# lkeegan/blockCG

Hardware: AMD Instinct MI355X
Metric: SBCGrQ lattice-site iterations/sec (iterations/sec x global volume), fp64 (higher is better)
Workload: dtype f64; 1 GPU; SBCGrQ V=64x64x64x64 (64x64x64x64 per GPU), m=16, 4 shifts, mass=0.001, fixed-work (eps=0); m=16, transport=none, half_volume_solves=False, memory_ladder_rung=whole tmp

## Files before the change

### blockcg_amd/csrc/capi_context.hip

```cpp
#include "capi_internal.hpp"

namespace bcg_impl {

std::string g_create_error;

void resolve_profile(bcg_context* c) {
  for (auto& kv : c->prof) {
    for (auto& pr : kv.second.pending) {
      float ms = 0.f;
      if (hipEventElapsedTime(&ms, pr.first, pr.second) == hipSuccess) {
        kv.second.ms += ms;
        kv.second.count += 1;
      }
      c->event_pool.push_back(pr.first);
      c->event_pool.push_back(pr.second);
    }
    kv.second.pending.clear();
  }
}

int stream_sync(bcg_context* c) {
  HIP_TRY(c, hipStreamSynchronize(c->stream));
  c->mat_in_flight = 0;
  if (c->profiling) resolve_profile(c);
// ... 327 lines not shown
  c->lat.ndim = ndim;
  c->lat.V = V;
  for (int mu = 0; mu < 4; ++mu) {
    c->lat.face_sites[mu] = V / c->lat.L[mu];
    c->lat.ghost_off[mu][0] = c->lat.ghost_off[mu][1] = 0;
    if (c->lat.split[mu]) {
      c->lat.ghost_off[mu][0] = ghost;
      c->lat.ghost_off[mu][1] = ghost + c->lat.face_sites[mu];
      ghost += 2 * c->lat.face_sites[mu];
    }
  }
  c->ghost_sites = ghost;
  if (const char* e = std::getenv("BCG_ROW_BLOCKS_B")) c->row_blocks_B = std::atoi(e);
  if (const char* e = std::getenv("BCG_ROW_BLOCKS_C")) c->row_blocks_C = std::atoi(e);
  if (const char* e = std::getenv("BCG_ROW_BATCHED")) c->row_batched = std::atoi(e) != 0;
  if (const char* e = std::getenv("BCG_HOP_WALK")) c->hop_tune.patch_walk = std::atoi(e) != 0;
  if (const char* e = std::getenv("BCG_HOP_BLOCKS")) c->hop_tune.blocks = std::atoi(e);
  if (const char* e = std::getenv("BCG_HOP_BLOCKS_OVERLAP")) c->hop_tune.blocks_overlap = std::atoi(e);
  if (const char* e = std::getenv("BCG_HOP_SUPER")) c->hop_tune.super_patch = std::atoi(e);
  if (const char* e = std::getenv("BCG_HOP_SYNC")) c->hop_tune.sync.window = std::atoi(e);
  if (const char* e = std::getenv("BCG_HOP_SYNC_LIMIT")) c->hop_tune.sync.limit_ticks = std::atoi(e);
  if (const char* e = std::getenv("BCG_HOP_COLUMN")) c->hop_tune.sync.column_walk = std::atoi(e) != 0;
  if (const char* e = std::getenv("BCG_HOP_BUNDLE")) c->hop_tune.sync.bundle_walk = std::atoi(e);
  if (const char* e = std::getenv("BCG_HOP_BUNDLE_SYNC")) c->hop_tune.sync.bundle_window = std::atoi(e);
  if (const char* e = std::getenv("BCG_LAZY_Q")) c->lazy_q = std::atoi(e);
  if (const char* e = std::getenv("BCG_PAIR_SHIFTS")) c->pair_shifts = std::atoi(e);
  if (const char* e = std::getenv("BCG_DEFER_X0")) c->defer_x0 = std::atoi(e) != 0;
  if (const char* e = std::getenv("BCG_DEBUG_X0_COND_LIMIT")) c->x0_cond_limit = std::atof(e);
  if (const char* e = std::getenv("BCG_RING_CHUNK")) c->ring_chunk_override = std::atoi(e);
  if (const char* e = std::getenv("BCG_DEBUG_FIELD_BUDGET")) c->debug_field_budget = static_cast<size_t>(std::atoll(e));
// ... 90 lines not shown
  if (!c) return BCG_ERR_INVALID;
  if (send) *send = c->halo_send;
  if (recv) *recv = c->halo_recv;
  if (bytes_each) *bytes_each = c->halo_bytes;
  return BCG_OK;
}

int bcg_debug_read_scratch(bcg_context* c, void* host, size_t bytes) {
  DeviceScope on_device(c);
  if (!c || !host || !c->partials || bytes > c->partials_bytes) return BCG_ERR_INVALID;
  BCG_TRY(stream_sync(c));
  HIP_TRY(c, hipMemcpy(host, c->partials, bytes, hipMemcpyDeviceToHost));
  return BCG_OK;
}

int bcg_context_stream(const bcg_context* c, void** stream_out, int* device_out) {
  if (!c) return BCG_ERR_INVALID;
  if (stream_out) *stream_out = c->stream;
  if (device_out) *device_out = c->device;
  return BCG_OK;
}

int bcg_overlap_tuning(bcg_context* c, int interior_blocks) {
  if (!c || interior_blocks < 0 || interior_blocks > kMaxGramBlocks / 2) return BCG_ERR_INVALID;
  if (interior_blocks > 0) c->hop_tune.blocks_overlap = interior_blocks;
  return BCG_OK;
}

int bcg_synchronize(bcg_context* c) {
  DeviceScope on_device(c);
// ... 325 lines not shown
```

### blockcg_amd/csrc/capi_internal.hpp

```cpp
#pragma once
#include <hip/hip_runtime.h>

#include <algorithm>
#include <cmath>
#include <cstdio>
#include <cstdlib>
#include <cstring>
#include <sstream>
#include <string>
#include <thread>
#include <vector>

#include "context.hpp"
#include "kernels_mfma.hpp"

#define BCG_FAIL(ctx, code, msg) \
  do {                           \
    (ctx)->err = (msg);          \
    return (code);               \
  } while (0)

#define HIP_TRY(ctx, call)                                                                         \
  do {                                                                                             \
    hipError_t e_ = (call);                                                                        \
// ... 20 lines not shown
  explicit DeviceScope(const bcg_context* c) {
    if (!c) return;
    if (hipGetDevice(&prev) == hipSuccess && prev != c->device) switched = hipSetDevice(c->device) == hipSuccess;
  }
  ~DeviceScope() {
    if (switched) (void)hipSetDevice(prev);
  }
  DeviceScope(const DeviceScope&) = delete;
  DeviceScope& operator=(const DeviceScope&) = delete;
};

struct ProfScope {
  bcg_context* c;
  bcg::ProfEntry* e = nullptr;
  hipEvent_t a = nullptr, b = nullptr;
  ProfScope(bcg_context* ctx, const char* name, double alg_bytes = 0.0, double alg_flops = 0.0) : c(ctx) {
    if (!c->profiling) return;
    e = &c->prof[name];
    e->bytes += alg_bytes;
    e->flops += alg_flops;
    a = take();
    b = take();
    (void)hipEventRecord(a, c->stream);
  }
  ~ProfScope() {
    if (!e) return;
    (void)hipEventRecord(b, c->stream);
    e->pending.emplace_back(a, b);
  }
  hipEvent_t take() {
    if (!c->event_pool.empty()) {
      hipEvent_t ev = c->event_pool.back();
      c->event_pool.pop_back();
      return ev;
    }
    hipEvent_t ev;
    (void)hipEventCreate(&ev);
    return ev;
  }
};

constexpr int kMaxGramBlocks = 2048;
constexpr size_t kMatSlotBytes = 32 * 32 * sizeof(double2);
constexpr int kMatSlots = 96;

constexpr int kFastBlocks = 1024;

inline int64_t rows_of(const bcg_field* f) { return f->sites * 3; }
inline double alg_bytes(const bcg_context* c, int m, double fields, double links = 0.0, int64_t num = 1, int64_t den = 1) {
  return static_cast<double>(c->lat.V) * (fields * 48.0 * m + links * 144.0 * c->ndim) * static_cast<double>(num) /
         static_cast<double>(den);
}
inline double row_bytes(const bcg_field* f, double fields) { return static_cast<double>(f->sites) * 48.0 * f->m * fields; }
inline double product_flops(const bcg_field* f, double products) {
  return static_cast<double>(f->sites) * 3.0 * f->m * f->m * 8.0 * products;
}
inline double hop_flops(const bcg_context* c, int m, bool gram, int64_t num = 1, int64_t den = 1) {
  return static_cast<double>(c->lat.V) * m * (72.0 * 2 * c->ndim + (gram ? 24.0 * m : 0.0)) * static_cast<double>(num) /
         static_cast<double>(den);
}
inline size_t field_bytes(const bcg_context* c, int m) { return static_cast<size_t>(c->lat.V) * 3 * m * sizeof(double2); }
// ... 21 lines not shown

int halo_plan(int ndim, const int* gdims, const int* grid, const int* coords, size_t site_bytes, int* peer_s, int* peer_r,
              size_t* off_s, size_t* off_r, size_t* nb, int64_t* ghost_sites);
inline bool can_overlap(const bcg_context* c) {
  return c->distributed && c->have_comm && c->comm.halo_exchange_begin && c->comm.halo_exchange_end;
}
int halo_field(bcg_context* c, const bcg_field* f, bool split = false);
int halo_gauge(bcg_context* c, bcg_gauge* g);
int hop(bcg_context* c, const bcg_gauge* g, bcg_field* out, const bcg_field* in, bcg::HopMode mode, const bcg_field* p, double c0,
        int* gram_blocks = nullptr, bool* gram_folded = nullptr);
int get_tmp(bcg_context* c, int m, bcg_field** out);
bool capacity_path(const bcg_context* c, int m);
inline bool ring_overlapped(const bcg_context* c) { return c->ring_overlap && can_overlap(c) && (c->tmp_ring - 2) / 2 >= 1; }
int reserve_operator_scratch(bcg_context* c, const bcg_field* like);
int apply_shifted(bcg_context* c, const bcg_gauge* g, double mass, double sigma0, bcg_field* T, const bcg_field* P,
                  int* gram_blocks = nullptr, bool* gram_folded = nullptr);

int pair_shifts_depth(const bcg_context* c, int m, int n_shifts);
int thin_qr(bcg_context* c, bcg_field* y, CMat& R);

}
```

### blockcg_amd/csrc/capi_operator.hip

```cpp
#include "capi_internal.hpp"

namespace bcg_impl {

int rank_of_grid(const int* grid, const int* xyz) {
  int r = 0, st = 1;
  for (int mu = 0; mu < 4; ++mu) {
    r += xyz[mu] * st;
    st *= grid[mu];
  }
  return r;
}

int halo_plan(int ndim, const int* gdims, const int* grid, const int* coords, size_t site_bytes, int* peer_s, int* peer_r,
              size_t* off_s, size_t* off_r, size_t* nb, int64_t* ghost_sites) {
  int g4[4] = {1, 1, 1, 1}, c4[4] = {0, 0, 0, 0}, L[4] = {1, 1, 1, 1};
  int64_t V = 1;
  for (int mu = 0; mu < ndim; ++mu) {
    g4[mu] = grid ? grid[mu] : 1;
    c4[mu] = coords ? coords[mu] : 0;
    if (g4[mu] < 1 || gdims[mu] < 1 || gdims[mu] % g4[mu] != 0 || c4[mu] < 0 || c4[mu] >= g4[mu]) return -1;
    L[mu] = gdims[mu] / g4[mu];
    V *= L[mu];
  }
  int n = 0;
// ... 445 lines not shown
  const int m = like->m;
  bcg_field* tmp;
  if (like->parity >= 0) {
    BCG_TRY(get_tmp_half(c, m, 1 - like->parity, &tmp));
    if (c->distributed) BCG_TRY(ensure_halo(c, static_cast<size_t>(c->ghost_sites) * 3 * m * sizeof(double2)));
    if (half_chunked_path(c) && fast_hop(c, m)) BCG_TRY(ensure_half_chunk_scratch(c, m));
    return BCG_OK;
  }
  if (fast_hop(c, m)) BCG_TRY(ensure_scratch(c));
  if (capacity_path(c, m)) return ensure_ring_scratch(c, m);
  BCG_TRY(get_tmp(c, m, &tmp));
  if (c->distributed) BCG_TRY(ensure_halo(c, static_cast<size_t>(c->ghost_sites) * 3 * m * sizeof(double2)));
  return BCG_OK;
}

int apply_shifted(bcg_context* c, const bcg_gauge* g, double mass, double sigma0, bcg_field* T, const bcg_field* P,
                  int* gram_blocks, bool* gram_folded) {
  if (gram_folded) *gram_folded = false;
  if (P->parity >= 0) {
    if (gram_blocks) *gram_blocks = 0;
    if (T->parity != P->parity) BCG_FAIL(c, BCG_ERR_INVALID, "half-volume operator: result and argument must have the same parity");
    const int m = P->m;
    bcg_field* tmp;
    BCG_TRY(get_tmp_half(c, m, 1 - P->parity, &tmp));
    BCG_TRY(halo_gauge(c, const_cast<bcg_gauge*>(g)));
    bcg::LatticeDev latc = c->lat;
    latc.L[0] /= 2;
    latc.V /= 2;
    for (int mu = 1; mu < 4; ++mu) latc.stride[mu] /= 2;
    for (int mu = 0; mu < 4; ++mu) {
      latc.face_sites[mu] /= 2;
      latc.ghost_off[mu][0] /= 2;
      latc.ghost_off[mu][1] /= 2;
// ... 56 lines not shown
      ProfScope ps(c, "hop_half", alg_bytes(c, m, 2, 2, 1, 2), hop_flops(c, m, false, 1, 2));
      bcg::launch_hop_half(c->stream, m, c->lat, tmp->parity, g->U, g->Ughost, P->d, c->halo_recv, tmp->d, bcg::HOP_PLAIN, nullptr, 0.0);
    }
    BCG_TRY(check_launch(c, "hop_half"));
    BCG_TRY(halo_field(c, tmp));
    {
      ProfScope ps(c, "hop_half_shifted", alg_bytes(c, m, 3, 2, 1, 2), hop_flops(c, m, false, 1, 2));
      bcg::launch_hop_half(c->stream, m, c->lat, T->parity, g->U, g->Ughost, tmp->d, c->halo_recv, T->d, bcg::HOP_SHIFTED, P->d,
                           mass * mass + sigma0);
    }
    return check_launch(c, "hop_half_shifted");
  }
  if (capacity_path(c, P->m)) return apply_shifted_ring(c, g, mass, sigma0, T, P, gram_blocks);
  bcg_field* tmp;
  BCG_TRY(get_tmp(c, P->m, &tmp));
  BCG_TRY(hop(c, g, tmp, P, bcg::HOP_PLAIN, nullptr, 0.0));
  return hop(c, g, T, tmp, bcg::HOP_SHIFTED, P, mass * mass + sigma0, gram_blocks, gram_folded);
}


}

using namespace bcg_impl;

extern "C" {

int bcg_halo_plan(int ndim, const int* global_dims, const int* grid, const int* coords, size_t site_bytes, int* peer_send,
                  int* peer_recv, size_t* send_offset, size_t* recv_offset, size_t* nbytes, int64_t* ghost_sites) {
  if (ndim < 1 || ndim > 4 || !global_dims || !peer_send || !peer_recv || !send_offset || !recv_offset || !nbytes) return -1;
  return halo_plan(ndim, global_dims, grid, coords, site_bytes, peer_send, peer_recv, send_offset, recv_offset, nbytes,
                   ghost_sites);
}
// ... 72 lines not shown
```

### blockcg_amd/csrc/capi_solvers.hip

```cpp
#include "capi_internal.hpp"

namespace bcg_impl {

int phase_A(bcg_context* c, const bcg_gauge* g, double mass, double sigma0, bcg_field* T, const bcg_field* P, CMat& G) {
  int nb = 0;
  bool folded = false;
  BCG_TRY(apply_shifted(c, g, mass, sigma0, T, P, &nb, &folded));
  if (nb > 0) return finish_gram(c, P->m, nb, G, true, folded);
  return gram(c, P, T, G);
}

int rmul(bcg_context* c, bcg_field* y, const bcg_field* x, const CMat& M, double b, bcg::RmulMode mode, const char* name);
bool lazy_q_width(const bcg_context* c, int m) {
  return c->lazy_q && fast_rows(c, m) && fast_rmul(c, m) && (m == 8 || m == 16 || (m == 32 && c->lazy_q > 1));
}

int phase_B(bcg_context* c, bcg_field* Q, const bcg_field* T, const CMat& alpha, CMat& G2, const CMat* rinv_prev = nullptr,
            bcg_field* Qout = nullptr) {
  const int m = Q->m;
  if (!fast_rows(c, m)) {
    if (Qout) BCG_FAIL(c, BCG_ERR_INVALID, "phase B: a separate output needs the fused kernel");
    BCG_TRY(rmul(c, Q, T, -alpha, 0.0, bcg::RMUL_ADD, "block_axpy"));
    return gram(c, Q, Q, G2);
  }
// ... 872 lines not shown
```

### blockcg_amd/csrc/context.hpp

```cpp
#pragma once
#include <hip/hip_runtime.h>

#include <map>
#include <string>
#include <vector>

#include "../../include/blockcg_hip.h"
#include "kernels.hpp"
#include "kernels_mfma.hpp"
#include "small_matrix.hpp"

struct bcg_field {
  bcg_context* ctx;
  int m;
  double2* d;
  void* base;
  int parity = -1;
  int64_t sites = 0;
};

struct bcg_gauge {
  bcg_context* ctx;
  double2* U;
  double2* Ughost;
// ... 18 lines not shown
  bool own_stream = false;
  int ndim = 1;
  int gdims[4] = {1, 1, 1, 1};
  int grid[4] = {1, 1, 1, 1};
  int coords[4] = {0, 0, 0, 0};
  bcg::LatticeDev lat{};
  int64_t ghost_sites = 0;
  bool distributed = false;
  bcg_comm comm{};
  bool have_comm = false;
  bool force_generic = false;
  bool force_tile_classes = false;
  int row_blocks_B = 1024, row_blocks_C = 1024;
  bool row_batched = true;
  bcg::HopTuning hop_tune;

  std::map<int, bcg_field*> tmp_field;
  int tmp_ring = 0;
  std::map<int, double2*> tmp_ring_buf;
  std::map<int, std::pair<int*, int>> boundary_tiles;
  double2* halo_send = nullptr;
  double2* halo_recv = nullptr;
  size_t halo_bytes = 0;
  void* halo_save = nullptr;
  size_t halo_save_bytes = 0;
  int lazy_q = 1;
  int pair_shifts = 4;
  bool defer_x0 = true;
  double x0_cond_limit = 64.0;
  size_t debug_field_budget = 0;
// ... 31 lines not shown
```

### blockcg_amd/csrc/kernels.hpp

```cpp
#pragma once
#include <hip/hip_runtime.h>

#include <cstdint>

namespace bcg {

struct LatticeDev {
  int ndim;
  int L[4];
  int origin[4];
  int split[4];
  int64_t V;
  int64_t stride[4];
  int64_t ghost_off[4][2];
  int64_t face_sites[4];
};

bool width_supported(int m);
bool mfma_width(int m);

void launch_axpby(hipStream_t s, double2* y, double a, const double2* x, double b, int64_t n);
void launch_scg_update(hipStream_t s, const double2* r, int nshift, double2* const* x, double2* const* p,
                       const double* alpha, const double* beta, const double* zeta, int64_t n);
void launch_host_to_dev(hipStream_t s, int m, const double2* host_layout, double2* dev_layout, int64_t nsites);
void launch_dev_to_host(hipStream_t s, int m, const double2* dev_layout, double2* host_layout, int64_t nsites);
void launch_fill_field(hipStream_t s, int m, const LatticeDev& lat, const int* gdims, double2* f, uint64_t seed);
void launch_fill_gauge(hipStream_t s, const LatticeDev& lat, const int* gdims, double2* U, uint64_t seed);

void launch_pack_faces(hipStream_t s, int m, const LatticeDev& lat, const double2* f, double2* send, int x3_lo = 0,
                       int x3_n = 0, int ring = 0);
void launch_pack_gauge_faces(hipStream_t s, const LatticeDev& lat, const double2* U, double2* send);

enum HopMode { HOP_PLAIN = 0, HOP_SHIFTED = 1, HOP_RESID = 2 };
void launch_hop_generic(hipStream_t s, int m, const LatticeDev& lat, const double2* U, const double2* Ughost,
                        const double2* in, const double2* ghost, double2* out, HopMode mode, const double2* p,
                        double c0);
void launch_pack_faces_half(hipStream_t s, int m, const LatticeDev& lat, int parity, const double2* f, double2* send,
                            int x3_lo = 0, int x3_n = 0);
void launch_hop_half(hipStream_t s, int m, const LatticeDev& lat, int parity, const double2* U, const double2* Ughost,
                     const double2* in, const double2* ghost, double2* out, HopMode mode, const double2* p, double c0);
void launch_parity_copy(hipStream_t s, int m, const LatticeDev& lat, int parity, double2* full, double2* half, bool to_half);
void launch_fill_field_half(hipStream_t s, int m, const LatticeDev& lat, const int* gdims, int parity, double2* f, uint64_t seed);

enum RmulMode { RMUL_ADD = 0, RMUL_XPAY = 1, RMUL_MUL = 2 };
void launch_rmul_generic(hipStream_t s, int m, int64_t rows, double2* y, const double2* x, const double2* Md,
                         double b, RmulMode mode);
void launch_trisolve_generic(hipStream_t s, int m, int64_t rows, double2* y, const double2* Rd);
int launch_gram_generic(hipStream_t s, int m, int64_t rows, const double2* a, const double2* b, double2* partials,
// ... 5 lines not shown
```

### blockcg_amd/csrc/kernels_mfma.hpp

```cpp
#pragma once
#include <hip/hip_runtime.h>

#include <cstdint>

#include "kernels.hpp"

namespace bcg {

bool mfma_rows_width(int m);
bool hop_fast_width(int m);
int phaseC_max_shifts(int m, bool applies_rinv);

struct GramFold {
  double2* out = nullptr;
  unsigned* tickets = nullptr;
};

int launch_phaseB(hipStream_t s, int m, int64_t rows, double2* Q, const double2* T, const double2* negalpha,
                  double2* partials, int max_blocks, bool batched, GramFold fold = GramFold(), const double2* rinv = nullptr,
                  double2* Qout = nullptr);
void launch_phaseC(hipStream_t s, int m, int64_t rows, double2* Q, double2* const* X, double2* const* P, int nshift,
                   const double2* mats, int apply_rinv, int max_blocks, double2* Y = nullptr);
bool phaseC_multi_fits(int m, int nsteps, int n_shifts);
int phaseC_multi_capacity(int m);
// ... 4 lines not shown
                      int max_blocks, bool batched);
void launch_rmul_mfma(hipStream_t s, int m, int64_t rows, double2* y, const double2* x, const double2* Cd, double b,
                      RmulMode mode, int max_blocks, bool batched);
int launch_gram_mfma(hipStream_t s, int m, int64_t rows, const double2* a, const double2* b, double2* partials,
                     int max_blocks);
struct HopSync {
  unsigned* counters = nullptr;
  int stride = 0;
  int window = 4;
  int limit_ticks = 5000;
  bool column_walk = true;
  int bundle_walk = 1;
  int bundle_window = 4;
};

struct HopTuning {
  bool patch_walk = true;
  int patch[3] = {0, 8, 8};
  int blocks = 512;
  HopSync sync;
  const int* boundary_list = nullptr;
  int boundary_n = 0;
  bool nontemporal = true;
  GramFold fold;
  int super_patch = 0;
  int blocks_overlap = 512;
};

struct HopWindow {
  int x3_lo = 0, x3_n = 0;
// ... 16 lines not shown
```

### blockcg_amd/csrc/kernels_stencil.hip

```cpp
#include "mfma_common.hpp"

namespace bcg {

namespace {

typedef __attribute__((address_space(3))) char lds_char_t;
__device__ __forceinline__ unsigned lds_addr_of(const void* p) {
  return static_cast<unsigned>(reinterpret_cast<uintptr_t>((lds_char_t*)p));
}
#ifndef BCG_HOP4B_PIPE
#define BCG_HOP4B_PIPE 1
#endif
#ifndef BCG_HOP4B_SPREAD
#define BCG_HOP4B_SPREAD 6
#endif
#ifndef BCG_HOP4B_BCAST
#define BCG_HOP4B_BCAST 1
#endif
__device__ __forceinline__ void glds16_link(const void* gsrc, unsigned lds_dst) {
  unsigned keep;
  asm volatile("s_mov_b32 %0, m0\n\ts_mov_b32 m0, %2\n\ts_nop 0\n\tglobal_load_lds_dwordx4 %1, off\n\ts_mov_b32 m0, %0"
               : "=&s"(keep)
               : "v"(gsrc), "s"(lds_dst));
}
// ... 750 lines not shown


__host__ __device__ constexpr bool hop4b_share_images(int m) { return m >= 16; }

template <int M, int MODE, bool GRAM, bool RING, bool CB = false>
__device__ __forceinline__ void hop4b_body(const LatticeDev& lat, const double2* __restrict__ U,
                                           const double2* __restrict__ Ughost, const double2* __restrict__ in,
                                           const double2* __restrict__ ghost, double2* __restrict__ out,
                                           const double2* __restrict__ p, double c0, double2* __restrict__ partials,
                                           const HopWalk& hw, const HopWindow& win) {
  static_assert(!GRAM || M == 16 || M == 8, "fused Gram accumulation: lane&15 = rhs index (m = 16) or (site parity, rhs) (m = 8)");
  constexpr bool RING_OUT = RING && MODE == HOP_PLAIN;
  constexpr bool RING_IN = RING && MODE == HOP_SHIFTED;
  constexpr bool RESID = MODE == HOP_RESID;
  static_assert(!RESID || (GRAM && !RING), "the residual form accumulates a Gram product and is not ring-addressed");
  static_assert(!CB || (!RING && !RESID), "checkerboard form: whole-field launches only");
  constexpr int SPW = 64 / M;
  constexpr int NW = 4;
  constexpr int CS = (SPW + 2) * 3 * M;
  constexpr int NFW = (SPW + 1) * 36;
  constexpr int NBW = (CB ? 4 : 3) * SPW * 9;
  constexpr int LSTAGE = NFW + NBW;
  constexpr int RFW = (SPW * 36 + 63) / 64;
  constexpr int RBK = (SPW * 9 + 63) / 64;
  constexpr bool SHARE = hop4b_share_images(M);
  constexpr bool PARTNER = SHARE && !CB;
  constexpr bool PIPE = BCG_HOP4B_PIPE != 0 && hop4b_share_images(M) && !RESID;
  constexpr int HB = 3 * M * 16;
  constexpr int NHD = (HB + 1023) / 1024;
  constexpr int RB = 3 * M * 16;
// ... 406 lines not shown
    if constexpr (PIPE) {
      dv2 q1[3], q2[3];
      {
        const char* const a1 = INCR_IN ? io_1 : row_o(k_o1, a_o1, s_o1, win.x3_lo, slot);
        const char* const a2 = INCR_IN ? io_2 : row_o(k_o2, a_o2, s_o2, win.x3_lo, slot);
        if (INCR_IN) { io_1 += id_o1; io_2 += id_o2; }
#pragma unroll
        for (int c = 0; c < 3; ++c) {
          const double2 v1 = ld_sv(a1, voff, c * M * 16), v2 = ld_sv(a2, voff, c * M * 16);
          q1[c] = dv2{v1.x, v1.y};
          q2[c] = dv2{v2.x, v2.y};
        }
        asm volatile("" : "+v"(q1[0]), "+v"(q1[1]), "+v"(q1[2]), "+v"(q2[0]), "+v"(q2[1]), "+v"(q2[2]));
      }
      constexpr int nB = 3 + 2 * NHD;
      constexpr int nE = MODE == HOP_PLAIN ? 0 : 3;
      const int nC = CB ? RFW + 4 * RBK : RFW + 1 + (e1 ? 0 : RBK) + (e2 ? 0 : RBK);
      constexpr int nD = 6, nS = 3;
      constexpr int SPREAD = MODE == HOP_PLAIN ? 0 : BCG_HOP4B_SPREAD;
      constexpr bool SP_B = (SPREAD & 1) != 0, SP_C = (SPREAD & 2) != 0, SP_D = (SPREAD & 4) != 0;
      (void)nB;
      for (int x3 = win.x3_lo; x3 < x3_end; ++x3) {
        const bool more = x3 + 1 < x3_end;
        const int slot_n = RING ? (slot + 1 == win.ring ? 0 : slot + 1) : 0;
        const int step_n = vs0 + x3;
        if (hw.sync != nullptr && tid == 0 && pace) {
          const int need = step_n - hw.sync_window;
          const unsigned known = seen2_idx == need ? seen2 : (seen1_idx == need ? seen1 : 0u);
          if (need >= 0 && known < per) {
            unsigned* ctr = hw.sync + cls * hw.sync_stride + need;
            const long long t0 = wall_clock64();
            while (read_counter(ctr, zero_rt) < per) {
              if (wall_clock64() - t0 > hw.sync_limit) {
                pace = false;
// ... 53 lines not shown
        glds16_s(b_rgt, fo + 1024, cn + (SPW + 1) * HB + 1024);                          \
      }                                                                                  \
    }                                                                                    \
  }
        BCG_ROW_PIECE(0)
        BCG_ROW_PIECE(1)
        if (!SP_B) { BCG_ROW_PIECE(2) BCG_ROW_PIECE(3) }
        BCG_STAMPB(2)
        const dv2* const Cown = Cc + wave * CS;
        const dv2* const Cp1 = Cc + (wave ^ 1) * CS;
        const dv2* const Cp2 = Cc + (wave ^ 2) * CS;
#pragma unroll
        for (int c = 0; c < 3; ++c) {
          f0[c] = Cown[co + (CB ? rr : 1) * 3 * M + c * M];
          b0[c] = Cown[co + (CB ? rr - 1 : -1) * 3 * M + c * M];
        }
        const int64_t crow_site = static_cast<int64_t>(col) + static_cast<int64_t>(x3) * S3;
        const char* const prow = INCR ? ip_p : reinterpret_cast<const char*>(p) + crow_site * RB;
        char* const orow = INCR_OUT ? ip_o : reinterpret_cast<char*>(out) + (RING_OUT ? static_cast<int64_t>(col) + static_cast<int64_t>(slot) * S3 : crow_site) * RB;
        if (INCR) ip_p += id_row;
        if (INCR_OUT) ip_o += id_row;
        dv2 pv[3], n1[3], n2[3];
        double2 acc[3] = {make_double2(0, 0), make_double2(0, 0), make_double2(0, 0)};
        const int x0 = CB ? 2 * (x0b + sw) + rr : x0b + sw;
        const int par1 = x0 + og0, par2 = par1 + x1 + og1, par3 = par2 + x2 + og2;
#define BCG_LD(K, UF, UB)                                                                                    \
  {                                                                                                          \
    _Pragma("unroll") for (int r = 0; r < 3; ++r) {                                                          \
      LU[r] = (UF)[(K) * 3 + r];                                                                             \
      LU[3 + r] = (UB)[r * 3 + (K)];                                                                         \
// ... 68 lines not shown
#pragma unroll
          for (int q = 0; q < 3; ++q) {
            const int e = l16 + 16 * q < 36 ? l16 + 16 * q : 35;
            LQ[q] = uf0[e];
            const int d = e / 9, i = e - 9 * d;
            const dv2* const ub = d == 0 ? ub0 : (d == 1 ? ub1 : (d == 2 ? ub2 : ub3));
            LQ[3 + q] = ub[i];
          }
        }
        __builtin_amdgcn_sched_barrier(0);
        BCG_PIPE_DIR(0, f0, b0, uf0, ub0, BCG_LD_LP(lp1, Cp1), if (SP_B) BCG_ROW_PIECE(2), if (SP_B) BCG_ROW_PIECE(3))
        BCG_PIPE_PIN;
        __builtin_amdgcn_sched_barrier(0);
#undef BCG_ROW_PIECE
        BCG_STAMPB(3)
        if (MODE != HOP_PLAIN) {
          asm volatile("; ASYNC_ISSUE p");
          pv[0] = ld_sv_async<0>(prow, voff);
          pv[1] = ld_sv_async<M * 16>(prow, voff);
          pv[2] = ld_sv_async<2 * M * 16>(prow, voff);
          asm volatile("; ASYNC_ISSUED p");
        }
        constexpr bool C_PIECES = SP_C && INCR && !CB;
        const unsigned imgn = __builtin_amdgcn_readfirstlane(lds_addr_of(image(x3 + 1, wave)));
#define BCG_LINK_PIECE(I)                                                                                    \
  if (more) {                                                                                                \
    if ((I) == 0) {                                                                                          \
      if (lane < SPW * 36) glds16_s(ik_f, fo, imgn + 36 * 16);                                               \
    }                                                                                                        \
    if ((I) == 1) {                                                                                          \
      if (RFW > 1 && lane + 64 < SPW * 36) glds16_s(ik_f, fo + 1024, imgn + (36 + 64) * 16);                 \
// ... 71 lines not shown
        BCG_PIPE_DIR(3, f3, b3, uf0 + 27, ub3, , , )
        BCG_PIPE_PIN;
        __builtin_amdgcn_sched_barrier(0);
#undef BCG_LD
#undef BCG_FM
#undef BCG_FM1
#undef BCG_FMB
#undef BCG_PIPE_DIR
#undef BCG_PIPE_SLOT
#undef BCG_LD_LP
#undef BCG_PIPE_PIN
#undef BCG_PIPE_APART
        BCG_STAMPB(9)
        if (more && !CB) park_u3(x3 + 1);
        double2 tv[3], pw[3];
        if (MODE != HOP_PLAIN) {
          wait_vmcnt(more ? nC + nD : 0);
          dv2 r0, r1, r2;
          asm volatile("; ASYNC_RETIRE p\n\tv_mov_b64 %0, %6\n\tv_mov_b64 %1, %7\n\tv_mov_b64 %2, %8\n\tv_mov_b64 %3, %9\n\tv_mov_b64 %4, %10\n\tv_mov_b64 %5, %11"
                       : "=&v"(r0.x), "=&v"(r0.y), "=&v"(r1.x), "=&v"(r1.y), "=&v"(r2.x), "=&v"(r2.y)
                       : "v"(pv[0].x), "v"(pv[0].y), "v"(pv[1].x), "v"(pv[1].y), "v"(pv[2].x), "v"(pv[2].y));
          pw[0] = make_double2(r0.x, r0.y);
          pw[1] = make_double2(r1.x, r1.y);
          pw[2] = make_double2(r2.x, r2.y);
        }
#pragma unroll
        for (int r = 0; r < 3; ++r) {
          if (MODE == HOP_PLAIN) tv[r] = make_double2(0.5 * acc[r].x, 0.5 * acc[r].y);
          else tv[r] = make_double2(fma(c0, pw[r].x, -0.5 * acc[r].x), fma(c0, pw[r].y, -0.5 * acc[r].y));
          st_nt(reinterpret_cast<double2*>(orow + voff + r * M * 16), tv[r]);
        }
        if (GRAM) {
#pragma unroll
          for (int r = 0; r < 3; ++r) gram_step<16>(G, &pw[r], &tv[r]);
        }
        BCG_STAMPB(10)
        __builtin_amdgcn_sched_barrier(0);
        if (more) {
          asm volatile("s_waitcnt vmcnt(%24) ; ASYNC_RETIRE n1 ASYNC_RETIRE n2\n\t"
                       "v_mov_b64 %0, %12\n\tv_mov_b64 %1, %13\n\tv_mov_b64 %2, %14\n\tv_mov_b64 %3, %15\n\tv_mov_b64 %4, %16\n\tv_mov_b64 %5, %17\n\t"
                       "v_mov_b64 %6, %18\n\tv_mov_b64 %7, %19\n\tv_mov_b64 %8, %20\n\tv_mov_b64 %9, %21\n\tv_mov_b64 %10, %22\n\tv_mov_b64 %11, %23"
                       : "=&v"(q1[0].x), "=&v"(q1[0].y), "=&v"(q1[1].x), "=&v"(q1[1].y), "=&v"(q1[2].x), "=&v"(q1[2].y),
                         "=&v"(q2[0].x), "=&v"(q2[0].y), "=&v"(q2[1].x), "=&v"(q2[1].y), "=&v"(q2[2].x), "=&v"(q2[2].y)
                       : "v"(n1[0].x), "v"(n1[0].y), "v"(n1[1].x), "v"(n1[1].y), "v"(n1[2].x), "v"(n1[2].y),
                         "v"(n2[0].x), "v"(n2[0].y), "v"(n2[1].x), "v"(n2[1].y), "v"(n2[2].x), "v"(n2[2].y), "n"(nS)
                       : "memory");
        } else {
          asm volatile("s_waitcnt vmcnt(%0)" : : "n"(nS) : "memory");
        }
// ... 73 lines not shown
          slice_of(x3 + 1, RING ? (slot + 1 == win.ring ? 0 : slot + 1) : 0, kind, xs, gx3);
          row_ptrs(kind, xs, gx3, own, hal);
        }
#pragma unroll
        for (int c = 0; c < 3; ++c) f[3][c] = ld_sv(own, voff, c * M * 16);
#pragma unroll
        for (int c = 0; c < 3; ++c)
          if (halo_lane) hv[c] = *reinterpret_cast<const dv2*>(hal + c * M * 16);
      }
      const int64_t crow_site = static_cast<int64_t>(col) + static_cast<int64_t>(x3) * S3;
      const char* const prow = INCR ? ip_p : reinterpret_cast<const char*>(p) + crow_site * RB;
      char* const orow = INCR_OUT ? ip_o : reinterpret_cast<char*>(out) + (RING_OUT ? static_cast<int64_t>(col) + static_cast<int64_t>(slot) * S3 : crow_site) * RB;
      if (INCR) ip_p += id_row;
      if (INCR_OUT) ip_o += id_row;
      double2 pv[3], bv[3];
      if (MODE != HOP_PLAIN) {
#pragma unroll
        for (int r = 0; r < 3; ++r) pv[r] = ld_nt(reinterpret_cast<const double2*>(prow + voff + r * M * 16));
      }
      if (RESID) {
#pragma unroll
        for (int r = 0; r < 3; ++r) bv[r] = ld_nt(reinterpret_cast<const double2*>(orow + voff + r * M * 16));
      }
      BCG_STAMPB(2)
      const dv2* const Cown = Cc + wave * CS;
      const dv2* const Cp1 = Cc + (wave ^ 1) * CS;
      const dv2* const Cp2 = Cc + (wave ^ 2) * CS;
#pragma unroll
      for (int c = 0; c < 3; ++c) {
        const dv2 a = Cown[co + (CB ? rr : 1) * 3 * M + c * M], b = Cown[co + (CB ? rr - 1 : -1) * 3 * M + c * M];
        f[0][c] = make_double2(a.x, a.y);
        bk[0][c] = make_double2(b.x, b.y);
      }
      constexpr bool DIRBRANCH = !GRAM;
      double2 lp1[3], lp2[3];
      if (DIRBRANCH) {
#pragma unroll
        for (int c = 0; c < 3; ++c) {
          const dv2 v1 = Cp1[co + c * M], v2 = Cp2[co + c * M];
          lp1[c] = make_double2(v1.x, v1.y);
          lp2[c] = make_double2(v2.x, v2.y);
        }
      } else {
        if (e1) {
#pragma unroll
          for (int c = 0; c < 3; ++c) { const dv2 v = Cp1[co + c * M]; f[1][c] = o1[c]; bk[1][c] = make_double2(v.x, v.y); }
        } else {
// ... 64 lines not shown
        else park_links(x3 + 1, false);
      }
      {
#pragma unroll
        for (int c = 0; c < 3; ++c) {
          dv2 v;
          v.x = f[3][c].x;
          v.y = f[3][c].y;
          Cn[co + c * M] = v;
          if (halo_lane) Cn[ho + c * M] = hv[c];
        }
      }
      double2 tv[3];
#pragma unroll
      for (int r = 0; r < 3; ++r) {
        if (MODE == HOP_PLAIN) tv[r] = make_double2(0.5 * acc[r].x, 0.5 * acc[r].y);
        else tv[r] = make_double2(fma(c0, pv[r].x, -0.5 * acc[r].x), fma(c0, pv[r].y, -0.5 * acc[r].y));
        if (RESID) tv[r] = make_double2(tv[r].x - bv[r].x, tv[r].y - bv[r].y);
        else st_nt(reinterpret_cast<double2*>(orow + voff + r * M * 16), tv[r]);
      }
      if (GRAM) {
#pragma unroll
        for (int r = 0; r < 3; ++r) gram_step<16>(G, RESID ? &tv[r] : &pv[r], &tv[r]);
      }
      if (hw.sync != nullptr && tid == 0 && step_n < hw.sync_stride)
        __hip_atomic_fetch_add(hw.sync + cls * hw.sync_stride + step_n, 1u, __ATOMIC_RELAXED, __HIP_MEMORY_SCOPE_AGENT);
      seen2 = seen1;
      seen2_idx = seen1_idx;
      if (hw.sync != nullptr && tid == 0 && pace && step_n + 2 >= hw.sync_window) {
        seen1_idx = step_n + 2 - hw.sync_window;
        seen1 = read_counter(hw.sync + cls * hw.sync_stride + seen1_idx, zero_rt);
      }
      if (RING) slot = slot + 1 == win.ring ? 0 : slot + 1;
      BCG_STAMPB(7)
    }
  }
#ifdef BCG_HOP4B_STAMPS
  if (!GRAM && lane == 0) {
    double* o = reinterpret_cast<double*>(partials) + (static_cast<int64_t>(blockIdx.x) * 4 + wave) * 16;
    for (int i = 0; i < 16; ++i) o[i] = static_cast<double>(seg[i]);
  }
#endif
#undef BCG_STAMPB
  if (GRAM) {
    if (M == 8) gram_block_store_fold8<NW>(G, smem, partials, tid, hw.fold.out != nullptr);
    else gram_block_store<16, NW>(G, smem, partials, tid, hw.fold.out != nullptr);
    gram_fold<M * M>(hw.fold, partials, tid, NW * 64);
  }
#undef BO_F
#undef BO_SEL
}

template <int M, int MODE, bool GRAM, bool RING, bool CB = false>
__global__ void __launch_bounds__(256) __attribute__((amdgpu_waves_per_eu(2, 2))) k_hop4b(
    LatticeDev lat, const double2* __restrict__ U, const double2* __restrict__ Ughost, const double2* __restrict__ in,
    const double2* __restrict__ ghost, double2* __restrict__ out, const double2* __restrict__ p, double c0,
    double2* __restrict__ partials, HopWalk hw, HopWindow win) {
  hop4b_body<M, MODE, GRAM, RING, CB>(lat, U, Ughost, in, ghost, out, p, c0, partials, hw, win);
}

#ifdef BCG_PROBE
template __global__ void k_hop4b<16, HOP_PLAIN, false, false>(LatticeDev, const double2*, const double2*, const double2*,
                                                               const double2*, double2*, const double2*, double, double2*,
                                                               HopWalk, HopWindow);
template __global__ void k_hop4b<16, HOP_SHIFTED, true, false>(LatticeDev, const double2*, const double2*, const double2*,
                                                                const double2*, double2*, const double2*, double, double2*,
                                                                HopWalk, HopWindow);
template __global__ void k_hop4c<16, HOP_PLAIN, false, 0, false>(LatticeDev, const double2*, const double2*, const double2*,
                                                                  const double2*, double2*, const double2*, double, double2*,
                                                                  HopWalk, HopWindow);
template __global__ void k_hop4c<16, HOP_SHIFTED, true, 0, false>(LatticeDev, const double2*, const double2*, const double2*,
                                                                   const double2*, double2*, const double2*, double, double2*,
                                                                   HopWalk, HopWindow);
}
}
#else
}

bool hop_fast_width(int m) { return m == 8 || m == 16 || m == 32; }
bool hop_can_split_tiles(int m, const LatticeDev& lat) {
  const int spb = 4 * (64 / m);
  return hop_fast_width(m) && lat.ndim == 4 && lat.L[0] % spb == 0 && lat.V < (int64_t(1) << 31) - 2 * lat.stride[3];
// ... 63 lines not shown

template <int M>
static int launch_hop4(hipStream_t s, const LatticeDev& lat, const double2* U, const double2* Ughost, const double2* in,
                       const double2* ghost, double2* out, HopMode mode, const double2* p, double c0, double2* partials,
                       bool gram, int max_blocks, const HopTuning& tune, int cls, const HopWindow& win_in) {
  constexpr int SPB = 4 * (64 / M);
  const HopPlan pl = plan_hop4(M, lat, max_blocks, tune, cls, win_in);
  if (!pl.valid) return -1;
  const int grid = pl.grid, ntiles = pl.ntiles;
  HopWalk hw = pl.hw;
  if (gram && pl.column && cls == 0) hw.fold = tune.fold;
  const HopWindow win = pl.win;
  const size_t lds_g = gram ? sizeof(double) * 4 * 8 * 64 : 0;
  if (pl.list && grid == 0) return 0;
  const int cls_t = pl.list ? 0 : cls;
  if (win.cb) {
    if (!hop4b_share_images(M) || (gram && M != 16) || mode == HOP_RESID || win.ring > 0 || cls != 0 || lat.split[0] ||
        !bundle_ok(M, lat, tune, pl, cls, true))
      return -1;
    constexpr int MC = hop4b_share_images(M) ? M : 16;
    HopWalk hwb = hw;
    if (tune.sync.bundle_window != 0 && hw.sync && (tune.sync.bundle_window < 0 || bundle_paced(M, ntiles, grid, win)))
      hwb.sync_window = tune.sync.bundle_window < 0 ? -tune.sync.bundle_window : tune.sync.bundle_window;
    else hwb.sync = nullptr;
    if (hwb.sync) (void)hipMemsetAsync(hwb.sync, 0, sizeof(unsigned) * 8 * hwb.sync_stride, s);
    constexpr int SPWc = 64 / MC;
    const size_t lds_u = sizeof(double2) * (2 * 4 * ((SPWc + 2) * 3 * MC) + 2 * 4 * ((SPWc + 1) * 36 + 4 * SPWc * 9));
    const size_t lds = lds_u > lds_g ? lds_u : lds_g;
#define BCG_LAUNCH4B_CB(MM, MD, GR)                                                                                      \
  do {                                                                                                              \
// ... 19 lines not shown
    const size_t lds = lds_u > lds_g ? lds_u : lds_g;
#define BCG_LAUNCH4B(MM, MD, GR, RG)                                                                                \
  do {                                                                                                             \
    allow_lds(k_hop4b<MM, MD, GR, RG>, lds);                                                                       \
    hipLaunchKernelGGL((k_hop4b<MM, MD, GR, RG>), dim3(grid), dim3(256), lds, s, lat, U, Ughost, in, ghost, out, p, \
                       c0, partials, hwb, win);                                                                     \
  } while (0)
#define BCG_LAUNCH4B_R(MM, MD, GR)                      \
  do {                                                  \
    if (win.ring > 0) BCG_LAUNCH4B(MM, MD, GR, true);   \
    else BCG_LAUNCH4B(MM, MD, GR, false);               \
  } while (0)
    if (mode == HOP_RESID) {
      if (M != 16 || !gram || win.ring > 0) return -1;
      BCG_LAUNCH4B(16, HOP_RESID, true, false);
    } else if (gram && M == 16 && mode == HOP_SHIFTED) BCG_LAUNCH4B_R(16, HOP_SHIFTED, true);
    else if (gram && M == 8 && mode == HOP_SHIFTED) BCG_LAUNCH4B_R(8, HOP_SHIFTED, true);
    else if (mode == HOP_PLAIN) BCG_LAUNCH4B_R(M, HOP_PLAIN, false);
    else BCG_LAUNCH4B_R(M, HOP_SHIFTED, false);
#undef BCG_LAUNCH4B_R
#undef BCG_LAUNCH4B
    return grid;
  }
  if (mode == HOP_RESID) return -1;
  if (pl.column) {
    if (hw.sync) (void)hipMemsetAsync(hw.sync, 0, sizeof(unsigned) * 8 * hw.sync_stride, s);
    const size_t lds_u = sizeof(double2) * 2 * ((SPB + 1) * 36 + 3 * SPB * 9);
    const size_t lds = lds_u > lds_g ? lds_u : lds_g;
#define BCG_LAUNCH4C(MM, MD, GR, CL, RG)                                                                                \
  do {                                                                                                                 \
    allow_lds(k_hop4c<MM, MD, GR, CL, RG>, lds);                                                                       \
    hipLaunchKernelGGL((k_hop4c<MM, MD, GR, CL, RG>), dim3(grid), dim3(256), lds, s, lat, U, Ughost, in, ghost, out, p, \
                       c0, partials, hw, win);                                                                         \
  } while (0)
#define BCG_LAUNCH4C_R(MM, MD, GR)                          \
  do {                                                      \
    if (win.ring > 0) BCG_LAUNCH4C(MM, MD, GR, 0, true);    \
    else if (cls == 1 && (GR || MM == 8)) {  \
      allow_lds(k_hop4c_interior<MM, MD, GR>, lds);         \
// ... 76 lines not shown
```

Baseline: 371.7 million site-iter/s.

## Factor shifted staggered operator into two first-order hops with self-Gram

Replaces the plain hop followed by the shifted hop (c0·P − D·D·P/4) with a factored pair, (μ − D/2) then (μ + D/2), where μ = sqrt(m² + σ). The first factor no longer needs a separate P read, and the second factor uses its own-site input, so the extra p-stream load and its async retire are dropped. The Gram product becomes tmpᴴ·tmp, which is Hermitian positive definite by construction; its diagonal is forced real. This changes the rounding behaviour of the operator. It is on by default and falls back to the unfactored path when the bundle kernel is unavailable.

```diff
diff --git a/blockcg_amd/csrc/capi_context.hip b/blockcg_amd/csrc/capi_context.hip
--- a/blockcg_amd/csrc/capi_context.hip
+++ b/blockcg_amd/csrc/capi_context.hip
@@ -365,6 +365,7 @@
   if (const char* e = std::getenv("BCG_ROW_BLOCKS_B")) c->row_blocks_B = std::atoi(e);
   if (const char* e = std::getenv("BCG_ROW_BLOCKS_C")) c->row_blocks_C = std::atoi(e);
   if (const char* e = std::getenv("BCG_ROW_BATCHED")) c->row_batched = std::atoi(e) != 0;
+  if (const char* e = std::getenv("BCG_HOP_FACTORED")) c->hop_factored = std::atoi(e) != 0;
   if (const char* e = std::getenv("BCG_HOP_WALK")) c->hop_tune.patch_walk = std::atoi(e) != 0;
   if (const char* e = std::getenv("BCG_HOP_BLOCKS")) c->hop_tune.blocks = std::atoi(e);
   if (const char* e = std::getenv("BCG_HOP_BLOCKS_OVERLAP")) c->hop_tune.blocks_overlap = std::atoi(e);
@@ -485,6 +486,12 @@
   return BCG_OK;
 }
 
+int bcg_debug_phase_a_gram(const bcg_context* c, int m, double* out) {
+  if (!c || !out || m <= 0 || c->phaseA_gram.dim() != m) return BCG_ERR_INVALID;
+  c->phaseA_gram.store(out);
+  return BCG_OK;
+}
+
 int bcg_context_stream(const bcg_context* c, void** stream_out, int* device_out) {
   if (!c) return BCG_ERR_INVALID;
   if (stream_out) *stream_out = c->stream;
diff --git a/blockcg_amd/csrc/capi_internal.hpp b/blockcg_amd/csrc/capi_internal.hpp
--- a/blockcg_amd/csrc/capi_internal.hpp
+++ b/blockcg_amd/csrc/capi_internal.hpp
@@ -58,14 +58,25 @@
   bcg_context* c;
   bcg::ProfEntry* e = nullptr;
   hipEvent_t a = nullptr, b = nullptr;
+  double booked_bytes = 0.0, booked_flops = 0.0;
   ProfScope(bcg_context* ctx, const char* name, double alg_bytes = 0.0, double alg_flops = 0.0) : c(ctx) {
     if (!c->profiling) return;
     e = &c->prof[name];
     e->bytes += alg_bytes;
     e->flops += alg_flops;
+    booked_bytes = alg_bytes;
+    booked_flops = alg_flops;
     a = take();
     b = take();
     (void)hipEventRecord(a, c->stream);
+  }
+  void cancel() {
+    if (!e) return;
+    e->bytes -= booked_bytes;
+    e->flops -= booked_flops;
+    c->event_pool.push_back(a);
+    c->event_pool.push_back(b);
+    e = nullptr;
   }
   ~ProfScope() {
     if (!e) return;
@@ -89,6 +100,9 @@
 constexpr int kMatSlots = 96;
 
 constexpr int kFastBlocks = 1024;
+static_assert(bcg::kHopStampsSkipBlocks == kFastBlocks &&
+                  static_cast<size_t>(bcg::kHopStampsSkipBlocks) * (32 * 32 * 16 + 4 * 16 * 8) <= static_cast<size_t>(kMaxGramBlocks) * 32 * 32 * 16,
+              "stamps of the Gram forms (4 waves x 16 doubles per block): behind the largest grid's partials, inside the buffer");
 
 inline int64_t rows_of(const bcg_field* f) { return f->sites * 3; }
 inline double alg_bytes(const bcg_context* c, int m, double fields, double links = 0.0, int64_t num = 1, int64_t den = 1) {
@@ -140,7 +154,7 @@
 inline bool ring_overlapped(const bcg_context* c) { return c->ring_overlap && can_overlap(c) && (c->tmp_ring - 2) / 2 >= 1; }
 int reserve_operator_scratch(bcg_context* c, const bcg_field* like);
 int apply_shifted(bcg_context* c, const bcg_gauge* g, double mass, double sigma0, bcg_field* T, const bcg_field* P,
-                  int* gram_blocks = nullptr, bool* gram_folded = nullptr);
+                  int* gram_blocks = nullptr, bool* gram_folded = nullptr, bool* gram_self = nullptr);
 
 int pair_shifts_depth(const bcg_context* c, int m, int n_shifts);
 int thin_qr(bcg_context* c, bcg_field* y, CMat& R);
diff --git a/blockcg_amd/csrc/capi_operator.hip b/blockcg_amd/csrc/capi_operator.hip
--- a/blockcg_amd/csrc/capi_operator.hip
+++ b/blockcg_amd/csrc/capi_operator.hip
@@ -483,9 +483,23 @@
   return BCG_OK;
 }
 
+static bool factored_pair(const bcg_context* c, int m, double c0, bool want_gram) {
+  if (!c->hop_factored || !want_gram || m != 16 || !(c0 > 0.0) || c->distributed || c->force_tile_classes || !fast_hop(c, m))
+    return false;
+  return bcg::hop_uses_bundle(m, c->lat, kFastBlocks, c->hop_tune, 0, bcg::HopWindow(), true) &&
+         bcg::hop_uses_bundle(m, c->lat, kFastBlocks, c->hop_tune, 0, bcg::HopWindow(), false);
+}
+
+static int apply_unfactored(bcg_context* c, const bcg_gauge* g, double mass, double sigma0, bcg_field* T, const bcg_field* P,
+                            bcg_field* tmp, int* gram_blocks, bool* gram_folded) {
+  BCG_TRY(hop(c, g, tmp, P, bcg::HOP_PLAIN, nullptr, 0.0));
+  return hop(c, g, T, tmp, bcg::HOP_SHIFTED, P, mass * mass + sigma0, gram_blocks, gram_folded);
+}
+
 int apply_shifted(bcg_context* c, const bcg_gauge* g, double mass, double sigma0, bcg_field* T, const bcg_field* P,
-                  int* gram_blocks, bool* gram_folded) {
+                  int* gram_blocks, bool* gram_folded, bool* gram_self) {
   if (gram_folded) *gram_folded = false;
+  if (gram_self) *gram_self = false;
   if (P->parity >= 0) {
     if (gram_blocks) *gram_blocks = 0;
     if (T->parity != P->parity) BCG_FAIL(c, BCG_ERR_INVALID, "half-volume operator: result and argument must have the same parity");
@@ -572,8 +586,38 @@
   if (capacity_path(c, P->m)) return apply_shifted_ring(c, g, mass, sigma0, T, P, gram_blocks);
   bcg_field* tmp;
   BCG_TRY(get_tmp(c, P->m, &tmp));
-  BCG_TRY(hop(c, g, tmp, P, bcg::HOP_PLAIN, nullptr, 0.0));
-  return hop(c, g, T, tmp, bcg::HOP_SHIFTED, P, mass * mass + sigma0, gram_blocks, gram_folded);
+  if (factored_pair(c, P->m, mass * mass + sigma0, gram_blocks != nullptr)) {
+    const double mu = std::sqrt(mass * mass + sigma0);
+    BCG_TRY(halo_gauge(c, const_cast<bcg_gauge*>(g)));
+    BCG_TRY(ensure_scratch(c));
+    bcg::HopTuning tune = c->hop_tune;
+    int nb1;
+    {
+      ProfScope ps(c, "hop", alg_bytes(c, P->m, 2, 1), hop_flops(c, P->m, false));
+      nb1 = bcg::launch_hop_fast(c->stream, P->m, c->lat, g->U, g->Ughost, P->d, c->halo_recv, tmp->d, bcg::HOP_FACT1, nullptr, mu,
+                                 c->partials, false, kFastBlocks, tune, 0);
+      if (nb1 < 0) ps.cancel();
+    }
+    if (nb1 < 0) return apply_unfactored(c, g, mass, sigma0, T, P, tmp, gram_blocks, gram_folded);
+    if (c->profiling) c->prof["stencil_form_factored_pair"].count += 1;
+    note_stencil_form(c, P->m, 0, bcg::HopWindow(), true);
+    BCG_TRY(check_launch(c, "hop"));
+    const bool fold = gram_folded && bcg::hop_folds_gram(P->m, c->lat, kFastBlocks, tune, bcg::HopWindow());
+    if (fold) tune.fold = bcg::GramFold{c->dev_gram, c->fold_tickets};
+    int nb;
+    {
+      note_stencil_form(c, P->m, 0, bcg::HopWindow());
+      ProfScope ps(c, "hop_shifted_gram", alg_bytes(c, P->m, 2, 1), hop_flops(c, P->m, true));
+      nb = bcg::launch_hop_fast(c->stream, P->m, c->lat, g->U, g->Ughost, tmp->d, c->halo_recv, T->d, bcg::HOP_FACT2, nullptr, mu,
+                                c->partials, true, kFastBlocks, tune, 0);
+    }
+    if (nb < 0) BCG_FAIL(c, BCG_ERR_UNSUPPORTED, "factored stencil pair: second factor rejected after the first ran");
+    *gram_blocks = nb;
+    if (fold) *gram_folded = true;
+    if (gram_self) *gram_self = true;
+    return check_launch(c, "hop_shifted_gram");
+  }
+  return apply_unfactored(c, g, mass, sigma0, T, P, tmp, gram_blocks, gram_folded);
 }
 
 
diff --git a/blockcg_amd/csrc/capi_solvers.hip b/blockcg_amd/csrc/capi_solvers.hip
--- a/blockcg_amd/csrc/capi_solvers.hip
+++ b/blockcg_amd/csrc/capi_solvers.hip
@@ -4,10 +4,18 @@
 
 int phase_A(bcg_context* c, const bcg_gauge* g, double mass, double sigma0, bcg_field* T, const bcg_field* P, CMat& G) {
   int nb = 0;
-  bool folded = false;
-  BCG_TRY(apply_shifted(c, g, mass, sigma0, T, P, &nb, &folded));
-  if (nb > 0) return finish_gram(c, P->m, nb, G, true, folded);
-  return gram(c, P, T, G);
+  bool folded = false, self = false;
+  BCG_TRY(apply_shifted(c, g, mass, sigma0, T, P, &nb, &folded, &self));
+  if (nb > 0) {
+    BCG_TRY(finish_gram(c, P->m, nb, G, true, folded));
+    if (self)
+      for (int i = 0; i < P->m; ++i) G(i, i) = G(i, i).real();
+    c->phaseA_gram = G;
+    return BCG_OK;
+  }
+  BCG_TRY(gram(c, P, T, G));
+  c->phaseA_gram = G;
+  return BCG_OK;
 }
 
 int rmul(bcg_context* c, bcg_field* y, const bcg_field* x, const CMat& M, double b, bcg::RmulMode mode, const char* name);
diff --git a/blockcg_amd/csrc/context.hpp b/blockcg_amd/csrc/context.hpp
--- a/blockcg_amd/csrc/context.hpp
+++ b/blockcg_amd/csrc/context.hpp
@@ -56,6 +56,8 @@
   int row_blocks_B = 1024, row_blocks_C = 1024;
   bool row_batched = true;
   bcg::HopTuning hop_tune;
+  bcg::CMat phaseA_gram;
+  bool hop_factored = true;
 
   std::map<int, bcg_field*> tmp_field;
   int tmp_ring = 0;
diff --git a/blockcg_amd/csrc/kernels.hpp b/blockcg_amd/csrc/kernels.hpp
--- a/blockcg_amd/csrc/kernels.hpp
+++ b/blockcg_amd/csrc/kernels.hpp
@@ -31,7 +31,7 @@
                        int x3_n = 0, int ring = 0);
 void launch_pack_gauge_faces(hipStream_t s, const LatticeDev& lat, const double2* U, double2* send);
 
-enum HopMode { HOP_PLAIN = 0, HOP_SHIFTED = 1, HOP_RESID = 2 };
+enum HopMode { HOP_PLAIN = 0, HOP_SHIFTED = 1, HOP_RESID = 2, HOP_FACT1 = 3, HOP_FACT2 = 4 };
 void launch_hop_generic(hipStream_t s, int m, const LatticeDev& lat, const double2* U, const double2* Ughost,
                         const double2* in, const double2* ghost, double2* out, HopMode mode, const double2* p,
                         double c0);
diff --git a/blockcg_amd/csrc/kernels_mfma.hpp b/blockcg_amd/csrc/kernels_mfma.hpp
--- a/blockcg_amd/csrc/kernels_mfma.hpp
+++ b/blockcg_amd/csrc/kernels_mfma.hpp
@@ -42,6 +42,8 @@
   int bundle_window = 4;
 };
 
+constexpr int kHopStampsSkipBlocks = 1024;
+
 struct HopTuning {
   bool patch_walk = true;
   int patch[3] = {0, 8, 8};
diff --git a/blockcg_amd/csrc/kernels_stencil.hip b/blockcg_amd/csrc/kernels_stencil.hip
--- a/blockcg_amd/csrc/kernels_stencil.hip
+++ b/blockcg_amd/csrc/kernels_stencil.hip
@@ -788,6 +788,11 @@
   constexpr bool RING_IN = RING && MODE == HOP_SHIFTED;
   constexpr bool RESID = MODE == HOP_RESID;
   static_assert(!RESID || (GRAM && !RING), "the residual form accumulates a Gram product and is not ring-addressed");
+  constexpr bool FACT = MODE == HOP_FACT1 || MODE == HOP_FACT2;
+  constexpr bool HAS_P = MODE == HOP_SHIFTED || MODE == HOP_RESID;
+  constexpr bool SHIFT = HAS_P || FACT;
+  static_assert(!FACT || (M == 16 && !RING && !CB), "factored pair: whole full-volume fields at m = 16");
+  static_assert(!FACT || GRAM == (MODE == HOP_FACT2), "factored pair: the second factor carries the Gram product");
   static_assert(!CB || (!RING && !RESID), "checkerboard form: whole-field launches only");
   constexpr int SPW = 64 / M;
   constexpr int NW = 4;
@@ -1224,10 +1229,10 @@
         asm volatile("" : "+v"(q1[0]), "+v"(q1[1]), "+v"(q1[2]), "+v"(q2[0]), "+v"(q2[1]), "+v"(q2[2]));
       }
       constexpr int nB = 3 + 2 * NHD;
-      constexpr int nE = MODE == HOP_PLAIN ? 0 : 3;
+      constexpr int nE = HAS_P ? 3 : 0;
       const int nC = CB ? RFW + 4 * RBK : RFW + 1 + (e1 ? 0 : RBK) + (e2 ? 0 : RBK);
       constexpr int nD = 6, nS = 3;
-      constexpr int SPREAD = MODE == HOP_PLAIN ? 0 : BCG_HOP4B_SPREAD;
+      constexpr int SPREAD = HAS_P ? BCG_HOP4B_SPREAD : 0;
       constexpr bool SP_B = (SPREAD & 1) != 0, SP_C = (SPREAD & 2) != 0, SP_D = (SPREAD & 4) != 0;
       (void)nB;
       for (int x3 = win.x3_lo; x3 < x3_end; ++x3) {
@@ -1311,6 +1316,11 @@
         for (int c = 0; c < 3; ++c) {
           f0[c] = Cown[co + (CB ? rr : 1) * 3 * M + c * M];
           b0[c] = Cown[co + (CB ? rr - 1 : -1) * 3 * M + c * M];
+        }
+        dv2 own[3];
+        if (FACT) {
+#pragma unroll
+          for (int c = 0; c < 3; ++c) own[c] = Cown[co + c * M];
         }
         const int64_t crow_site = static_cast<int64_t>(col) + static_cast<int64_t>(x3) * S3;
         const char* const prow = INCR ? ip_p : reinterpret_cast<const char*>(p) + crow_site * RB;
@@ -1409,7 +1419,7 @@
         __builtin_amdgcn_sched_barrier(0);
 #undef BCG_ROW_PIECE
         BCG_STAMPB(3)
-        if (MODE != HOP_PLAIN) {
+        if (HAS_P) {
           asm volatile("; ASYNC_ISSUE p");
           pv[0] = ld_sv_async<0>(prow, voff);
           pv[1] = ld_sv_async<M * 16>(prow, voff);
@@ -1511,7 +1521,7 @@
         BCG_STAMPB(9)
         if (more && !CB) park_u3(x3 + 1);
         double2 tv[3], pw[3];
-        if (MODE != HOP_PLAIN) {
+        if (HAS_P) {
           wait_vmcnt(more ? nC + nD : 0);
           dv2 r0, r1, r2;
           asm volatile("; ASYNC_RETIRE p\n\tv_mov_b64 %0, %6\n\tv_mov_b64 %1, %7\n\tv_mov_b64 %2, %8\n\tv_mov_b64 %3, %9\n\tv_mov_b64 %4, %10\n\tv_mov_b64 %5, %11"
@@ -1521,15 +1531,20 @@
           pw[1] = make_double2(r1.x, r1.y);
           pw[2] = make_double2(r2.x, r2.y);
         }
+        if (FACT) {
+#pragma unroll
+          for (int r = 0; r < 3; ++r) pw[r] = make_double2(own[r].x, own[r].y);
+        }
 #pragma unroll
         for (int r = 0; r < 3; ++r) {
-          if (MODE == HOP_PLAIN) tv[r] = make_double2(0.5 * acc[r].x, 0.5 * acc[r].y);
+          if (!SHIFT) tv[r] = make_double2(0.5 * acc[r].x, 0.5 * acc[r].y);
+          else if (MODE == HOP_FACT2) tv[r] = make_double2(fma(c0, pw[r].x, 0.5 * acc[r].x), fma(c0, pw[r].y, 0.5 * acc[r].y));
           else tv[r] = make_double2(fma(c0, pw[r].x, -0.5 * acc[r].x), fma(c0, pw[r].y, -0.5 * acc[r].y));
           st_nt(reinterpret_cast<double2*>(orow + voff + r * M * 16), tv[r]);
         }
         if (GRAM) {
 #pragma unroll
-          for (int r = 0; r < 3; ++r) gram_step<16>(G, &pw[r], &tv[r]);
+          for (int r = 0; r < 3; ++r) gram_step<16>(G, &pw[r], FACT ? &pw[r] : &tv[r]);
         }
         BCG_STAMPB(10)
         __builtin_amdgcn_sched_barrier(0);
@@ -1633,7 +1648,7 @@
       if (INCR) ip_p += id_row;
       if (INCR_OUT) ip_o += id_row;
       double2 pv[3], bv[3];
-      if (MODE != HOP_PLAIN) {
+      if (HAS_P) {
 #pragma unroll
         for (int r = 0; r < 3; ++r) pv[r] = ld_nt(reinterpret_cast<const double2*>(prow + voff + r * M * 16));
       }
@@ -1650,6 +1665,10 @@
         const dv2 a = Cown[co + (CB ? rr : 1) * 3 * M + c * M], b = Cown[co + (CB ? rr - 1 : -1) * 3 * M + c * M];
         f[0][c] = make_double2(a.x, a.y);
         bk[0][c] = make_double2(b.x, b.y);
+        if (FACT) {
+          const dv2 o = Cown[co + c * M];
+          pv[c] = make_double2(o.x, o.y);
+        }
       }
       constexpr bool DIRBRANCH = !GRAM;
       double2 lp1[3], lp2[3];
@@ -1744,14 +1763,15 @@
       double2 tv[3];
 #pragma unroll
       for (int r = 0; r < 3; ++r) {
-        if (MODE == HOP_PLAIN) tv[r] = make_double2(0.5 * acc[r].x, 0.5 * acc[r].y);
+        if (!SHIFT) tv[r] = make_double2(0.5 * acc[r].x, 0.5 * acc[r].y);
+        else if (MODE == HOP_FACT2) tv[r] = make_double2(fma(c0, pv[r].x, 0.5 * acc[r].x), fma(c0, pv[r].y, 0.5 * acc[r].y));
         else tv[r] = make_double2(fma(c0, pv[r].x, -0.5 * acc[r].x), fma(c0, pv[r].y, -0.5 * acc[r].y));
         if (RESID) tv[r] = make_double2(tv[r].x - bv[r].x, tv[r].y - bv[r].y);
         else st_nt(reinterpret_cast<double2*>(orow + voff + r * M * 16), tv[r]);
       }
       if (GRAM) {
 #pragma unroll
-        for (int r = 0; r < 3; ++r) gram_step<16>(G, RESID ? &tv[r] : &pv[r], &tv[r]);
+        for (int r = 0; r < 3; ++r) gram_step<16>(G, RESID ? &tv[r] : &pv[r], FACT ? &pv[r] : &tv[r]);
       }
       if (hw.sync != nullptr && tid == 0 && step_n < hw.sync_stride)
         __hip_atomic_fetch_add(hw.sync + cls * hw.sync_stride + step_n, 1u, __ATOMIC_RELAXED, __HIP_MEMORY_SCOPE_AGENT);
@@ -1766,8 +1786,8 @@
     }
   }
 #ifdef BCG_HOP4B_STAMPS
-  if (!GRAM && lane == 0) {
-    double* o = reinterpret_cast<double*>(partials) + (static_cast<int64_t>(blockIdx.x) * 4 + wave) * 16;
+  if ((!GRAM || FACT) && lane == 0) {
+    double* o = reinterpret_cast<double*>(partials) + (GRAM ? kHopStampsSkipBlocks * M * M * 2 : 0) + (static_cast<int64_t>(blockIdx.x) * 4 + wave) * 16;
     for (int i = 0; i < 16; ++i) o[i] = static_cast<double>(seg[i]);
   }
 #endif
@@ -1796,6 +1816,12 @@
 template __global__ void k_hop4b<16, HOP_SHIFTED, true, false>(LatticeDev, const double2*, const double2*, const double2*,
                                                                 const double2*, double2*, const double2*, double, double2*,
                                                                 HopWalk, HopWindow);
+template __global__ void k_hop4b<16, HOP_FACT1, false, false>(LatticeDev, const double2*, const double2*, const double2*,
+                                                               const double2*, double2*, const double2*, double, double2*,
+                                                               HopWalk, HopWindow);
+template __global__ void k_hop4b<16, HOP_FACT2, true, false>(LatticeDev, const double2*, const double2*, const double2*,
+                                                              const double2*, double2*, const double2*, double, double2*,
+                                                              HopWalk, HopWindow);
 template __global__ void k_hop4c<16, HOP_PLAIN, false, 0, false>(LatticeDev, const double2*, const double2*, const double2*,
                                                                   const double2*, double2*, const double2*, double, double2*,
                                                                   HopWalk, HopWindow);
@@ -1889,6 +1915,8 @@
   const size_t lds_g = gram ? sizeof(double) * 4 * 8 * 64 : 0;
   if (pl.list && grid == 0) return 0;
   const int cls_t = pl.list ? 0 : cls;
+  const bool fact = mode == HOP_FACT1 || mode == HOP_FACT2;
+  if (fact && (M != 16 || win.cb || win.ring > 0 || cls != 0 || gram != (mode == HOP_FACT2))) return -1;
   if (win.cb) {
     if (!hop4b_share_images(M) || (gram && M != 16) || mode == HOP_RESID || win.ring > 0 || cls != 0 || lat.split[0] ||
         !bundle_ok(M, lat, tune, pl, cls, true))
@@ -1938,7 +1966,9 @@
     if (mode == HOP_RESID) {
       if (M != 16 || !gram || win.ring > 0) return -1;
       BCG_LAUNCH4B(16, HOP_RESID, true, false);
-    } else if (gram && M == 16 && mode == HOP_SHIFTED) BCG_LAUNCH4B_R(16, HOP_SHIFTED, true);
+    } else if (mode == HOP_FACT1) BCG_LAUNCH4B(16, HOP_FACT1, false, false);
+    else if (mode == HOP_FACT2) BCG_LAUNCH4B(16, HOP_FACT2, true, false);
+    else if (gram && M == 16 && mode == HOP_SHIFTED) BCG_LAUNCH4B_R(16, HOP_SHIFTED, true);
     else if (gram && M == 8 && mode == HOP_SHIFTED) BCG_LAUNCH4B_R(8, HOP_SHIFTED, true);
     else if (mode == HOP_PLAIN) BCG_LAUNCH4B_R(M, HOP_PLAIN, false);
     else BCG_LAUNCH4B_R(M, HOP_SHIFTED, false);
@@ -1946,7 +1976,7 @@
 #undef BCG_LAUNCH4B
     return grid;
   }
-  if (mode == HOP_RESID) return -1;
+  if (mode == HOP_RESID || fact) return -1;
   if (pl.column) {
     if (hw.sync) (void)hipMemsetAsync(hw.sync, 0, sizeof(unsigned) * 8 * hw.sync_stride, s);
     const size_t lds_u = sizeof(double2) * 2 * ((SPB + 1) * 36 + 3 * SPB * 9);
```

Result: faster. 381.3 million site-iter/s (median of 6 runs) (+2.6%).
